# conroi/lcpc

Hardware: AMD Instinct MI355X
Metric: field-elements committed/sec (whole node), Ligero 2^26 coeffs (higher is better)
Workload: dtype u32 limbs (255-bit prime field Ft255, Montgomery form)

## Files before the change

### lcpc_amd/csrc/ntt_l9s.hip

```cpp
#include "kernels.h"
#include "ntt_ln_dev.h"

namespace lcpc {

namespace {

template <bool M2> struct Tw { LN<9> b0, b1; };
template <> struct Tw<false> { LN<9> b0; };
template <bool M2, u32 NV> LCPC_DEV Tw<M2> tw_get(const u32* blk, u32 period, u32 variant, u32 jl) {
  using FT = LnField<FT255>;
  Tw<M2> t;
  if constexpr (M2) {
    t.b0 = pack_get<FT, 2 * NV>(blk, period, variant, jl);
    t.b1 = pack_get<FT, 2 * NV>(blk, period, NV + variant, jl);
  } else {
    t.b0 = pack_get<FT, NV>(blk, period, variant, jl);
  }
  return t;
}
template <bool M2> LCPC_DEV LN<9> tw_mul(const LN<9>& x, const Tw<M2>& w) {
  if constexpr (M2) return ln::mul2<LnField<FT255>>(x, w.b0, w.b1);
  else return ln::mul<LnField<FT255>>(x, w.b0);
}

template <int S, int LTJ, bool FIRST, bool MID, bool NF, bool M2>
__global__ void __launch_bounds__(256, 4) ntt_pass_l9s_kernel(NttPassArgs a, const u32* __restrict__ pack, NttPackInfo pi) {
  using FT = LnField<FT255>;
  constexpr int NL = 8, LT = S + LTJ, LBT = LTJ;
  constexpr bool LAST = !FIRST;
  static_assert(LT == 10, "1024-element tiles: one radix-4 quad (two radix-2 pairs) per thread and round");
  static_assert(FIRST || (LTJ == 0 && S % 2 == 0), "the last pass works on contiguous tiles and ends with the trivial stages k-2, k-1");
  static_assert(NF || !M2, "the two-table multiply serves the pure / coset form only");
  using SH = Shape<S, LBT>;
  using SP = PureShape<S>;
  constexpr int RU = NF ? (FIRST ? SP::RU : -1) : SH::RU;
  constexpr int RC = NF && FIRST ? SP::RC : -1;
  constexpr bool SWZD = NF ? (LAST || SP::RU >= 0) : RU >= 0;
  auto SWZ = [](u32 e) -> u32 {
    if constexpr (NF && LAST) return e ^ (((e >> 4) & 3u) * 5u);
    else if constexpr (NF && FIRST && SWZD && LBT == 2) return e ^ ((((e >> 4) ^ (e >> 6)) & 3u) << 2);
    else if constexpr (SWZD) return e ^ ((e >> 4) & 15u);
    else return e;
  };
  extern __shared__ __attribute__((aligned(16))) u32 lds[];
  constexpr u32 T = 1u << LT;
  u32* nqp = lds + (size_t)T * 9;
  const u32 k = a.log_n;
  const u32 tiles_per_row = 1u << (k - LT);
  u64 row;
  u32 tile;
  if (FIRST && a.tile_group) {
    const u32 lg = a.tile_group;
    const u32 xcd = blockIdx.x & 7u;
    const u64 qq = blockIdx.x >> 3;
    const u32 sub = (u32)qq & ((1u << lg) - 1);
    const u64 q2 = qq >> lg;
    tile = (((u32)(q2 / a.n_rows) * 8u + xcd) << lg) | sub;
    row = q2 % a.n_rows;
  } else if (tiles_per_row >= 8) {
    const u32 xcd = blockIdx.x & 7u;
    const u64 qq = blockIdx.x >> 3;
    tile = (u32)(qq / a.n_rows) * 8u + xcd;
    row = qq % a.n_rows;
  } else {
    row = blockIdx.x / tiles_per_row;
    tile = blockIdx.x % tiles_per_row;
  }
  const u32 tid = threadIdx.x;
  mem_phase(true);
  const u32 lb = FIRST ? k - S : 0u;
  auto gindex = [&](u32 e) -> u32 {
    if constexpr (FIRST) return ((e >> LBT) << lb) | (tile << LTJ) | (e & ((1u << LBT) - 1));
    else return (tile << S) | e;
  };
  const bool canon = a.roots29c != nullptr && ((u32)row & a.canon_row_mask) == 0;
  for (u32 i = tid; i < 64 * 12; i += 256) nqp[i] = 0u - a.qp29[i];
  const u32* src = a.src + row * a.src_stride * NL;
  constexpr bool DIRECT = !(LAST && MID);
  LN<9> xin[4];
  if constexpr (LAST && MID) {
    const uint4* t4 = reinterpret_cast<const uint4*>(a.mid + (row << k) * 9 + (size_t)tile * (9 * T));
    uint4* l4 = reinterpret_cast<uint4*>(lds);
    if constexpr (SWZD) {
#pragma unroll
      for (u32 i = tid; i < 2 * T; i += 256) l4[(i & ~(T - 1)) | SWZ(i & (T - 1))] = t4[i];
#pragma unroll
      for (u32 i = tid; i < T / 4; i += 256) {
        const uint4 v = t4[2 * T + i];
        const u32 b = 8 * T + SWZ(4 * i);
        lds[b] = v.x; lds[b ^ 1u] = v.y; lds[b ^ 2u] = v.z; lds[b ^ 3u] = v.w;
      }
    } else {
#pragma unroll
    for (u32 i = tid; i < 9 * T / 4; i += 256) l4[i] = t4[i];
    }
  } else {
#pragma unroll
  for (u32 it = 0; it < 4; it++) {
    const u32 e = tid + 256u * it;
    const u32 g = gindex(e);
    Fe<NL> v;
    if constexpr (FIRST) {
      v = (g < a.n_valid && row * a.src_stride + g < a.n_src_total) ? fe_load<NL>(src + (size_t)g * NL) : fe_zero<NL>();
      if (a.copy_dst != nullptr && g < a.n_valid) fe_store<NL>(a.copy_dst + (row * a.src_stride + g) * NL, v);
    } else {
      v = fe_load<NL>(src + (size_t)g * NL);
    }
    xin[it] = ln::from_packed<FT>(v);
  }
  __builtin_amdgcn_sched_barrier(0);
  }
  const u32* cls_pack = pack + (size_t)(FIRST != NF ? tile : 0u) * pi.class_words;
  const bool blk0_tile = (FIRST || tile == 0) && a.blk0_gone == 0;
  LN<9> k32;
#pragma unroll
  for (int i = 0; i < 9; i++) k32.v[i] = i == 0 ? 32u : 0u;
  const bool zero_hi = FIRST && a.n_valid <= (1ull << (k - 1));
  if constexpr (!DIRECT) __syncthreads();

  if constexpr (SH::U0 == 1) {
    constexpr u32 half = 1u << (S - 1 + LBT);
    const u32* blk = cls_pack + pi.round_off[0];
#pragma unroll
    for (u32 pp = 0; pp < 2; pp++) {
      const u32 e1 = tid + 256u * pp;
      const Tw<M2> w = NF ? tw_get<M2, 2>(blk, 1u << (S - 1), canon ? 1u : 0u, e1 >> LBT) : tw_get<M2, 2>(blk, SH::period2, canon ? 1u : 0u, e1);
      const LN<9> x = DIRECT ? xin[pp] : planes_get<FT>(lds, T, SWZ(e1));
      if (pp == 0) mem_phase(false);
      const bool cvs = NF && canon && SH::NR4 <= 1;
      if (zero_hi) {
        if constexpr (DIRECT) planes_put<FT>(lds, T, SWZ(e1), cvs ? ln::mul<FT>(x, k32) : x);
        planes_put<FT>(lds, T, SWZ(e1 + half), tw_mul<M2>(x, w));
      } else {
        const LN<9> y = DIRECT ? xin[pp + 2] : planes_get<FT>(lds, T, SWZ(e1 + half));
        LN<9> sum = ln::add(x, y);
        ln::normalize<FT>(sum);
        planes_put<FT>(lds, T, SWZ(e1), cvs ? ln::mul<FT>(sum, k32) : sum);
        planes_put<FT>(lds, T, SWZ(e1 + half), tw_mul<M2>(ln::sub(x, y), w));
      }
    }
    mem_phase(true);
    __syncthreads();
  }

  const u32 q = tid;
  if constexpr (NF && LAST) {
#pragma unroll
    for (int r = 0; r < 5; r++) {
      const int hb = 9 - 2 * r;
      const u32 D = 1u << (hb - 1);
      const u32 m = q >> (hb - 1);
      const u32 e0 = (m << (hb + 1)) | (q & (D - 1));
      const bool from_regs = DIRECT && r == 0;
      LN<9> x0 = from_regs ? xin[0] : planes_get<FT>(lds, T, SWZ(e0));
      const LN<9> x1 = from_regs ? xin[1] : planes_get<FT>(lds, T, SWZ(e0 + D));
      const LN<9> x2 = from_regs ? xin[2] : planes_get<FT>(lds, T, SWZ(e0 + 2 * D)), x3 = from_regs ? xin[3] : planes_get<FT>(lds, T, SWZ(e0 + 3 * D));
      LN<9> p1, p2, p3;
      if (r < 2) {
        const u32 sb = r == 0 ? 0u : (u32)__builtin_amdgcn_readfirstlane(tid >> 6);
        const u32* wu = cls_pack + pi.u_off + ((u32)r * 4 + sb) * (3 * U_SLOT<FT>);
        mem_phase(false);
        if (!from_regs) ln::clamp_apply<FT>(x0, ln::clamp_row<FT>(nqp, ln::clamp_q<FT>(x0.v[8])));
        p2 = ln::mul_u<FT>(x2, wu + U_SLOT<FT>);
        p1 = ln::mul_u<FT>(x1, wu);
        p3 = ln::mul_u<FT>(x3, wu + 2 * U_SLOT<FT>);
      } else {
        const u32* blk = cls_pack + pi.round_off[r];
        const Tw<M2> w1 = tw_get<M2, 3>(blk, coset_sets(r), 0, m), w2 = tw_get<M2, 3>(blk, coset_sets(r), 1, m);
        const Tw<M2> w3 = tw_get<M2, 3>(blk, coset_sets(r), 2, m);
        mem_phase(false);
        ln::clamp_apply<FT>(x0, ln::clamp_row<FT>(nqp, ln::clamp_q<FT>(x0.v[8])));
        p2 = tw_mul<M2>(x2, w2);
        p1 = tw_mul<M2>(x1, w1);
        p3 = tw_mul<M2>(x3, w3);
      }
      const LN<9> s02 = ln::add(x0, p2), d02 = ln::sub(x0, p2), s13 = ln::add(p1, p3);
      LN<9> y0 = ln::add(s02, s13), y1 = ln::sub(s02, s13);
      ln::normalize<FT>(y0);
      const LN<9> t = ln::mul_u<FT>(ln::sub(p1, p3), a.wq_w);
      LN<9> y2 = ln::add(d02, t), y3 = ln::sub(d02, t);
      if (r == 0 || r == 4) { ln::normalize<FT>(y1); ln::normalize<FT>(y2); ln::normalize<FT>(y3); }
      mem_phase(true);
      if (r < 4) {
        planes_put<FT>(lds, T, SWZ(e0), y0);
        planes_put<FT>(lds, T, SWZ(e0 + D), y1);
        planes_put<FT>(lds, T, SWZ(e0 + 2 * D), y2);
        planes_put<FT>(lds, T, SWZ(e0 + 3 * D), y3);
        __syncthreads();
      } else {
        u32* dstq = a.dst + row * a.dst_stride * NL + (size_t)((tile << S) | e0) * NL;
        LN<9> cc[4] = {y0, y1, y2, y3};
#pragma unroll
        for (int c = 0; c < 4; c++) {
          LN<9> x = cc[c];
          ln::clamp_apply<FT>(x, ln::clamp_row<FT>(nqp, ln::clamp_q<FT>(x.v[8])));
          u32 w[8];
          ln::to_packed<FT>(w, x.v);
          Fe<NL> v;
#pragma unroll
          for (int i = 0; i < 8; i++) v.v[i] = w[i];
          if (__any((int)(x.v[8] >= FT::limb(8)))) v = fe_reduce_once<8>(w);
          fe_store<NL>(dstq + (size_t)c * NL, v);
        }
      }
    }
    return;
  }
#pragma unroll
  for (int r = 0; r < SH::NR4; r++) {
    const int u = SH::U0 + 2 * r, hb = S - u - 1;
    const bool last_two = LAST && (r == SH::NR4 - 1);
    const bool triv = NF && FIRST && (r == SH::NR4 - 1);
    const u32 lp = q & ((1u << LBT) - 1), j = q >> LBT;
    const u32 i0 = ((j >> (hb - 1)) << (hb + 1)) | (j & ((1u << (hb - 1)) - 1));
    const u32 e0 = (i0 << LBT) | lp;
    constexpr u32 one = 1u;
    const u32 dq = one << (hb - 1 + LBT);
    const u32 period = NF ? one << (hb - 1) : one << (hb - 1 + LBT);
    const u32 jl = NF ? j & (period - 1) : q & (period - 1);
    const u32* blk = cls_pack + pi.round_off[SH::U0 + r];
    if (triv) {
      const bool fr = DIRECT && SH::U0 == 0 && r == 0;
      const LN<9> x0 = fr ? xin[0] : planes_get<FT>(lds, T, SWZ(e0)), x1 = fr ? xin[1] : planes_get<FT>(lds, T, SWZ(e0 + dq));
      const LN<9> x2 = fr ? xin[2] : planes_get<FT>(lds, T, SWZ(e0 + 2 * dq)), x3 = fr ? xin[3] : planes_get<FT>(lds, T, SWZ(e0 + 3 * dq));
      mem_phase(false);
      const LN<9> b0 = ln::add(x0, x2), b1 = ln::add(x1, x3);
      LN<9> c0 = ln::add(b0, b1), c1 = ln::sub(b0, b1);
      const LN<9> b2 = ln::sub(x0, x2);
      const LN<9> t = ln::mul_u<FT>(ln::sub(x1, x3), a.wq_w);
      LN<9> c2 = ln::add(b2, t), c3 = ln::sub(b2, t);
      ln::normalize<FT>(c1); ln::normalize<FT>(c2); ln::normalize<FT>(c3);
      if (RC < 0 && SH::U0 == 0 && canon) {
        ln::normalize<FT>(c0);
        c0 = ln::mul<FT>(c0, k32); c1 = ln::mul<FT>(c1, k32); c2 = ln::mul<FT>(c2, k32); c3 = ln::mul<FT>(c3, k32);
      } else if (fr) {
        ln::normalize<FT>(c0);
      } else {
        ln::clamp_apply<FT>(c0, ln::clamp_row<FT>(nqp, ln::clamp_q<FT>(c0.v[8])));
      }
      planes_put<FT>(lds, T, SWZ(e0), c0);
      planes_put<FT>(lds, T, SWZ(e0 + dq), c1);
      planes_put<FT>(lds, T, SWZ(e0 + 2 * dq), c2);
      planes_put<FT>(lds, T, SWZ(e0 + 3 * dq), c3);
      mem_phase(true);
      __syncthreads();
      continue;
    }
    if constexpr (RU >= 0) {
      if (r >= RU && !last_two) {
        const u32 wv = __builtin_amdgcn_readfirstlane(tid >> 6);
        const u32 qu = NF ? (((((tid & 63u) >> LBT) << 2) | wv) << LBT) | (tid & ((1u << LBT) - 1)) : ((tid & 63u) << 2) | wv;
        const u32 lpu = qu & ((1u << LBT) - 1), ju = qu >> LBT;
        const u32 iu = ((ju >> (hb - 1)) << (hb + 1)) | (ju & ((1u << (hb - 1)) - 1));
        const u32 eu = (iu << LBT) | lpu;
        const u32* wu = cls_pack + pi.u_off + ((r - RU) * 4 + wv) * (3 * U_SLOT<FT>);
        const LN<9> x0 = planes_get<FT>(lds, T, SWZ(eu)), x1 = planes_get<FT>(lds, T, SWZ(eu + dq));
        const LN<9> x2 = planes_get<FT>(lds, T, SWZ(eu + 2 * dq)), x3 = planes_get<FT>(lds, T, SWZ(eu + 3 * dq));
        mem_phase(false);
        const LN<9> b0 = ln::add(x0, x2), b1 = ln::add(x1, x3);
        LN<9> c0 = ln::add(b0, b1);
        ln::clamp_apply<FT>(c0, ln::clamp_row<FT>(nqp, ln::clamp_q<FT>(c0.v[8])));
        planes_put<FT>(lds, T, SWZ(eu), c0);
        LN<9> d1 = ln::sub(b0, b1);
        ln::normalize<FT>(d1);
        planes_put<FT>(lds, T, SWZ(eu + dq), ln::mul_u<FT>(d1, wu + 2 * U_SLOT<FT>));
        const LN<9> b2 = ln::mul_u<FT>(ln::sub(x0, x2), wu);
        const LN<9> b3 = ln::mul_u<FT>(ln::sub(x1, x3), wu + U_SLOT<FT>);
        LN<9> c2 = ln::add(b2, b3);
        if constexpr (NF) ln::clamp_apply<FT>(c2, ln::clamp_row<FT>(nqp, ln::clamp_q<FT>(c2.v[8])));
        else ln::normalize<FT>(c2);
        planes_put<FT>(lds, T, SWZ(eu + 2 * dq), c2);
        planes_put<FT>(lds, T, SWZ(eu + 3 * dq), ln::mul_u<FT>(ln::sub(b2, b3), wu + 2 * U_SLOT<FT>));
        mem_phase(true);
        __syncthreads();
        continue;
      }
    }
    if (u == 0 && zero_hi) {
      const u32 vb = canon ? 3u : 0u;
      const Tw<M2> w0 = tw_get<M2, 6>(blk, period, vb + 0, jl), w3 = tw_get<M2, 6>(blk, period, vb + 1, jl), w2 = tw_get<M2, 6>(blk, period, vb + 2, jl);
      mem_phase(false);
      const bool cv0 = NF && canon && r == RC;
      if (a.n_valid <= (1ull << (k - 2))) {
        const LN<9> x0 = DIRECT ? xin[0] : planes_get<FT>(lds, T, SWZ(e0));
        if constexpr (DIRECT) planes_put<FT>(lds, T, SWZ(e0), cv0 ? ln::mul<FT>(x0, k32) : x0);
        planes_put<FT>(lds, T, SWZ(e0 + dq), tw_mul<M2>(x0, w2));
        planes_put<FT>(lds, T, SWZ(e0 + 2 * dq), tw_mul<M2>(x0, w0));
        planes_put<FT>(lds, T, SWZ(e0 + 3 * dq), tw_mul<M2>(x0, w3));
      } else {
        const LN<9> x0 = DIRECT ? xin[0] : planes_get<FT>(lds, T, SWZ(e0)), x1 = DIRECT ? xin[1] : planes_get<FT>(lds, T, SWZ(e0 + dq));
        LN<9> c0 = ln::add(x0, x1);
        ln::normalize<FT>(c0);
        planes_put<FT>(lds, T, SWZ(e0), cv0 ? ln::mul<FT>(c0, k32) : c0);
        planes_put<FT>(lds, T, SWZ(e0 + dq), tw_mul<M2>(ln::sub(x0, x1), w2));
        const LN<9> t = ln::mul_u<FT>(x1, a.wq_w);
        planes_put<FT>(lds, T, SWZ(e0 + 2 * dq), tw_mul<M2>(ln::add(x0, t), w0));
        planes_put<FT>(lds, T, SWZ(e0 + 3 * dq), tw_mul<M2>(ln::sub(x0, t), w3));
      }
      mem_phase(true);
      __syncthreads();
      continue;
    }
    const bool from_regs = DIRECT && SH::U0 == 0 && r == 0;
    const LN<9> x0 = from_regs ? xin[0] : planes_get<FT>(lds, T, SWZ(e0)), x1 = from_regs ? xin[1] : planes_get<FT>(lds, T, SWZ(e0 + dq));
    const LN<9> x2 = from_regs ? xin[2] : planes_get<FT>(lds, T, SWZ(e0 + 2 * dq)), x3 = from_regs ? xin[3] : planes_get<FT>(lds, T, SWZ(e0 + 3 * dq));
    mem_phase(false);
    const LN<9> b0 = ln::add(x0, x2), b1 = ln::add(x1, x3);
    LN<9> c0 = ln::add(b0, b1);
    if (last_two) {
      ln::normalize<FT>(c0);
      LN<9> c1 = ln::sub(b0, b1);
      const LN<9> b2 = ln::sub(x0, x2);
      const LN<9> b3 = ln::mul_u<FT>(ln::sub(x1, x3), a.wq_w);
      LN<9> c2 = ln::add(b2, b3);
      LN<9> c3 = ln::sub(b2, b3);
      ln::normalize<FT>(c1); ln::normalize<FT>(c2); ln::normalize<FT>(c3);
      mem_phase(true);
      u32* dstq = a.dst + row * a.dst_stride * NL + (size_t)((tile << S) | e0) * NL;
      LN<9> cc[4] = {c0, c1, c2, c3};
#pragma unroll
      for (int c = 0; c < 4; c++) {
        LN<9> x = cc[c];
        ln::clamp_apply<FT>(x, ln::clamp_row<FT>(nqp, ln::clamp_q<FT>(x.v[8])));
        u32 w[8];
        ln::to_packed<FT>(w, x.v);
        Fe<NL> v;
#pragma unroll
        for (int i = 0; i < 8; i++) v.v[i] = w[i];
        if (__any((int)(x.v[8] >= FT::limb(8)))) v = fe_reduce_once<8>(w);
        fe_store<NL>(dstq + (size_t)c * NL, v);
      }
      return;
    } else {
      if (from_regs) ln::normalize<FT>(c0);
      else ln::clamp_apply<FT>(c0, ln::clamp_row<FT>(nqp, ln::clamp_q<FT>(c0.v[8])));
      planes_put<FT>(lds, T, SWZ(e0), c0);
      const bool blk0c = NF ? canon && q < dq : canon && blk0_tile && q < period && (RU < 0 || r < RU);
      if constexpr (NF ? RC >= 0 : RU >= 1) {
        if (r == (NF ? RC : RU - 1) && blk0c) {
          planes_put<FT>(lds, T, SWZ(e0), ln::mul<FT>(c0, k32));
        }
      }
      const u32 vb = blk0c ? 3u : 0u;
      if constexpr (M2) {
        const Tw<M2> w2 = tw_get<M2, 6>(blk, period, vb + 2, jl), w0 = tw_get<M2, 6>(blk, period, vb + 0, jl);
        const LN<9> d1 = ln::sub(b0, b1);
        const LN<9> d13 = ln::sub(x1, x3), e2 = ln::sub(x0, x2);
        planes_put<FT>(lds, T, SWZ(e0 + dq), tw_mul<M2>(d1, w2));
        __builtin_amdgcn_sched_barrier(0);
        const Tw<M2> w3 = tw_get<M2, 6>(blk, period, vb + 1, jl);
        const LN<9> t = ln::mul_u<FT>(d13, a.wq_w);
        planes_put<FT>(lds, T, SWZ(e0 + 2 * dq), tw_mul<M2>(ln::add(e2, t), w0));
        planes_put<FT>(lds, T, SWZ(e0 + 3 * dq), tw_mul<M2>(ln::sub(e2, t), w3));
      } else {
      const Tw<M2> w0 = tw_get<M2, 6>(blk, period, vb + 0, jl), w3 = tw_get<M2, 6>(blk, period, vb + 1, jl);
      const Tw<M2> w2 = tw_get<M2, 6>(blk, period, vb + 2, jl);
      const LN<9> d1 = ln::sub(b0, b1);
      planes_put<FT>(lds, T, SWZ(e0 + dq), tw_mul<M2>(d1, w2));
      const LN<9> t = ln::mul_u<FT>(ln::sub(x1, x3), a.wq_w);
      const LN<9> e2 = ln::sub(x0, x2);
      planes_put<FT>(lds, T, SWZ(e0 + 2 * dq), tw_mul<M2>(ln::add(e2, t), w0));
      planes_put<FT>(lds, T, SWZ(e0 + 3 * dq), tw_mul<M2>(ln::sub(e2, t), w3));
      }
    }
    mem_phase(true);
    __syncthreads();
  }

  if constexpr (FIRST && MID) {
    u32* mrow = a.mid + (row << k) * 9;
#pragma unroll
    for (u32 e = tid; e < T; e += 256) {
      const u32 e2 = (tile << LTJ) | (e & ((1u << LBT) - 1));
      u32* t = mrow + (size_t)(e >> LBT) * (9 * T);
      const LN<9> x = planes_get<FT>(lds, T, SWZ(e));
      *reinterpret_cast<uint4*>(t + (size_t)e2 * 4) = make_uint4(x.v[0], x.v[1], x.v[2], x.v[3]);
      *reinterpret_cast<uint4*>(t + (size_t)(T + e2) * 4) = make_uint4(x.v[4], x.v[5], x.v[6], x.v[7]);
      t[(size_t)8 * T + e2] = x.v[8];
    }
    return;
  }
  if constexpr (FIRST) {
  u32* dst = a.dst + row * a.dst_stride * NL;
#pragma unroll
  for (u32 e = tid; e < T; e += 256) {
    const u32 g = gindex(e);
    LN<9> x = planes_get<FT>(lds, T, SWZ(e));
    ln::clamp_apply<FT>(x, ln::clamp_row<FT>(nqp, ln::clamp_q<FT>(x.v[8])));
    u32 w[8];
    ln::to_packed<FT>(w, x.v);
    Fe<NL> v;
#pragma unroll
    for (int i = 0; i < 8; i++) v.v[i] = w[i];
    fe_store<NL>(dst + (size_t)g * NL, v);
  }
  }
}

template <int S, int LTJ, bool FIRST, bool MID, bool NF, bool M2>
hipError_t launch_tm(const NttPassArgs& a, const u32* pack, const NttPackInfo& pi, hipStream_t st) {
  constexpr int LT = S + LTJ;
  const u64 tiles = ((u64)1 << (a.log_n - LT)) * a.n_rows;
  const size_t lds_bytes = (((size_t)1 << LT) * 9 + 64 * LnField<FT255>::STRIDE) * 4;
  hipError_t e = hipFuncSetAttribute(reinterpret_cast<const void*>(&ntt_pass_l9s_kernel<S, LTJ, FIRST, MID, NF, M2>),
                                     hipFuncAttributeMaxDynamicSharedMemorySize, (int)lds_bytes);
  if (e != hipSuccess) return e;
  hipLaunchKernelGGL((ntt_pass_l9s_kernel<S, LTJ, FIRST, MID, NF, M2>), dim3((unsigned)tiles), dim3(256), lds_bytes, st, a, pack, pi);
  return hipGetLastError();
}
template <int S, int LTJ, bool FIRST>
hipError_t launch_t(const NttPassArgs& a, const u32* pack, const NttPackInfo& pi, hipStream_t st) {
  if (pi.mul2) {
    if constexpr (ntt_l9s_mul2_supported(S, FIRST)) { if (a.form) return a.mid ? launch_tm<S, LTJ, FIRST, true, true, true>(a, pack, pi, st) : launch_tm<S, LTJ, FIRST, false, true, true>(a, pack, pi, st); }
    return hipErrorInvalidValue;
  }
  if (a.form) return a.mid ? launch_tm<S, LTJ, FIRST, true, true, false>(a, pack, pi, st) : launch_tm<S, LTJ, FIRST, false, true, false>(a, pack, pi, st);
  return a.mid ? launch_tm<S, LTJ, FIRST, true, false, false>(a, pack, pi, st) : launch_tm<S, LTJ, FIRST, false, false, false>(a, pack, pi, st);
}

}

bool ntt_l9s3_supported(uint32_t log_n) { return log_n >= 21 && log_n <= 26; }

bool ntt_l9s_supported(uint32_t log_n, uint32_t n_passes, int log_tile) { return n_passes == 2 && log_tile == 10 && log_n >= 11 && log_n <= 20; }

#define L9S_FIRST_CASES(X) X(1) X(2) X(3) X(4) X(5) X(6) X(7) X(8) X(9) X(10)

hipError_t launch_ntt_pass_l9s(const NttPassArgs& a, bool first, const uint32_t* pack, const NttPackInfo& pi, hipStream_t st) {
  if (!first) {
    if (a.s != 10 || a.log_tj != 0 || a.t0 + a.s != a.log_n) return hipErrorInvalidValue;
    if (a.mont_prefix) return hipErrorInvalidValue;
    return launch_t<10, 0, false>(a, pack, pi, st);
  }
  if (a.t0 != 0 || a.s + a.log_tj != 10 || (a.s + 10 != a.log_n && a.s + 20 != a.log_n)) return hipErrorInvalidValue;
  if (a.form && a.s + 10 != a.log_n) return hipErrorInvalidValue;
  if (a.tile_group && ((1u << (a.log_n - 10)) >> a.tile_group) < 8) return hipErrorInvalidValue;
  switch (a.s) {
#define X(SV) case SV: return launch_t<SV, 10 - SV, true>(a, pack, pi, st);
    L9S_FIRST_CASES(X)
#undef X
  }
  return hipErrorInvalidValue;
}

}
```

### lcpc_amd/csrc/ntt_ln_dev.h

```cpp
#pragma once
#include "field_ln.h"

namespace lcpc {

template <int S, int LBT> struct Shape {
  static constexpr int U0 = S & 1;
  static constexpr int NR4 = S / 2;
  static constexpr u32 period2 = 1u << (S - 1 + LBT);
  static constexpr u32 period4(int r) { return 1u << (S - U0 - 2 * r - 2 + LBT); }
  static constexpr int RU = NR4 >= 4 ? 3 : -1;
  static constexpr int NRU = RU < 0 ? 0 : NR4 - RU;
};
template <int S> struct PureShape {
  static constexpr int U0 = S & 1;
  static constexpr int NR4 = S / 2;
  static constexpr u32 sets(int r) { return 1u << (S - U0 - 2 * r - 2); }
  static constexpr int RU = NR4 >= 3 ? NR4 - 2 : -1;
  static constexpr int RC = NR4 >= 3 ? NR4 - 3 : (NR4 == 2 ? 0 : -1);
};
constexpr u32 coset_sets(int r) { return 1u << (2 * r); }

template <class FT> constexpr u32 U_SLOT = (FT::N * FT::N + 31) & ~31u;
template <class FT> constexpr u32 U_ALIGN = FT::N == 9 ? 4u : 16u;

template <class FT, class C = u32> LCPC_DEV LN<FT::N> planes_get(const u32* base, C cnt, u32 e) {
  constexpr int N = FT::N;
  LN<N> r;
  if constexpr (N == 3) {
    const uint2 a = *reinterpret_cast<const uint2*>(base + (size_t)e * 2);
    r.v[0] = a.x; r.v[1] = a.y; r.v[2] = base[(size_t)cnt * 2 + e];
  } else {
    const uint4 a = *reinterpret_cast<const uint4*>(base + (size_t)e * 4);
    r.v[0] = a.x; r.v[1] = a.y; r.v[2] = a.z; r.v[3] = a.w;
    if constexpr (N == 5) {
      r.v[4] = base[(size_t)cnt * 4 + e];
    } else if constexpr (N == 7) {
      const uint2 b = *reinterpret_cast<const uint2*>(base + (size_t)cnt * 4 + (size_t)e * 2);
      r.v[4] = b.x; r.v[5] = b.y; r.v[6] = base[(size_t)cnt * 6 + e];
    } else {
      const uint4 b = *reinterpret_cast<const uint4*>(base + ((size_t)cnt + e) * 4);
      r.v[4] = b.x; r.v[5] = b.y; r.v[6] = b.z; r.v[7] = b.w; r.v[8] = base[(size_t)cnt * 8 + e];
    }
  }
  return r;
}
template <class FT, class C = u32> LCPC_DEV void planes_put(u32* base, C cnt, u32 e, const LN<FT::N>& x) {
  constexpr int N = FT::N;
  if constexpr (N == 3) {
    *reinterpret_cast<uint2*>(base + (size_t)e * 2) = make_uint2(x.v[0], x.v[1]);
    base[(size_t)cnt * 2 + e] = x.v[2];
  } else {
    *reinterpret_cast<uint4*>(base + (size_t)e * 4) = make_uint4(x.v[0], x.v[1], x.v[2], x.v[3]);
    if constexpr (N == 5) {
      base[(size_t)cnt * 4 + e] = x.v[4];
    } else if constexpr (N == 7) {
      *reinterpret_cast<uint2*>(base + (size_t)cnt * 4 + (size_t)e * 2) = make_uint2(x.v[4], x.v[5]);
      base[(size_t)cnt * 6 + e] = x.v[6];
    } else {
      *reinterpret_cast<uint4*>(base + ((size_t)cnt + e) * 4) = make_uint4(x.v[4], x.v[5], x.v[6], x.v[7]);
      base[(size_t)cnt * 8 + e] = x.v[8];
    }
  }
}

template <class FT> LCPC_DEV LN<FT::N> tab_entry(const u32* tab, u32 idx) {
  if constexpr (FT::STRIDE == 12) {
    return ln::load_limbs<FT::N>(tab + (size_t)idx * 12);
  } else {
    LN<FT::N> t;
#pragma unroll
    for (int k = 0; k < FT::N; k++) t.v[k] = tab[(size_t)idx * FT::STRIDE + k];
    return t;
  }
}

template <class FT, u32 NV> LCPC_DEV LN<FT::N> pack_get(const u32* blk, u32 period, u32 variant, u32 jl) {
  if constexpr (FT::N == 9) {
    const char* base = reinterpret_cast<const char*>(blk);
    const uint4 a = *reinterpret_cast<const uint4*>(base + (((variant * 2 + 0) * period + jl) << 4));
    const uint4 b = *reinterpret_cast<const uint4*>(base + (((variant * 2 + 1) * period + jl) << 4));
    const u32 c = *reinterpret_cast<const u32*>(base + ((NV * 2 * period * 4 + variant * period + jl) << 2));
    LN<9> t;
    t.v[0] = a.x; t.v[1] = a.y; t.v[2] = a.z; t.v[3] = a.w; t.v[4] = b.x; t.v[5] = b.y; t.v[6] = b.z; t.v[7] = b.w; t.v[8] = c;
    return t;
  } else {
    return planes_get<FT>(blk, NV * period, variant * period + jl);
  }
}
template <class FT, u32 NV> LCPC_DEV void pack_put(u32* blk, u32 period, u32 variant, u32 jl, const LN<FT::N>& x) {
  if constexpr (FT::N == 9) {
    *reinterpret_cast<uint4*>(blk + ((size_t)(variant * 2 + 0) * period + jl) * 4) = make_uint4(x.v[0], x.v[1], x.v[2], x.v[3]);
    *reinterpret_cast<uint4*>(blk + ((size_t)(variant * 2 + 1) * period + jl) * 4) = make_uint4(x.v[4], x.v[5], x.v[6], x.v[7]);
    blk[(size_t)NV * 2 * period * 4 + (size_t)variant * period + jl] = x.v[8];
  } else {
    planes_put<FT>(blk, NV * period, variant * period + jl, x);
  }
}

}
```

Measured before the change: 7.540 billion.

## Drop redundant normalizes before clamp-store and fuse trivial final round with global store

Removes normalize calls on outputs that are immediately clamped and stored, relying on clamp_store to bring values into range. Adds a path where the trivial (twiddle-free) last radix-4 round in non-MID configurations writes directly to global memory via gindex instead of going through LDS and another pass. Factors the clamp/pack/reduce/store sequence into a shared clamp_store helper. This saves ALU work and an LDS round trip, but correctness depends on clamp bounds tolerating unnormalized inputs, and the extra path without reduction must still yield canonical values.

```diff
diff --git a/lcpc_amd/csrc/ntt_l9s.hip b/lcpc_amd/csrc/ntt_l9s.hip
--- a/lcpc_amd/csrc/ntt_l9s.hip
+++ b/lcpc_amd/csrc/ntt_l9s.hip
@@ -176,10 +176,10 @@
       }
       const LN<9> s02 = ln::add(x0, p2), d02 = ln::sub(x0, p2), s13 = ln::add(p1, p3);
       LN<9> y0 = ln::add(s02, s13), y1 = ln::sub(s02, s13);
-      ln::normalize<FT>(y0);
+      if (r < 4) ln::normalize<FT>(y0);
       const LN<9> t = ln::mul_u<FT>(ln::sub(p1, p3), a.wq_w);
       LN<9> y2 = ln::add(d02, t), y3 = ln::sub(d02, t);
-      if (r == 0 || r == 4) { ln::normalize<FT>(y1); ln::normalize<FT>(y2); ln::normalize<FT>(y3); }
+      if (r == 0) { ln::normalize<FT>(y1); ln::normalize<FT>(y2); ln::normalize<FT>(y3); }
       mem_phase(true);
       if (r < 4) {
         planes_put<FT>(lds, T, SWZ(e0), y0);
@@ -189,19 +189,10 @@
         __syncthreads();
       } else {
         u32* dstq = a.dst + row * a.dst_stride * NL + (size_t)((tile << S) | e0) * NL;
-        LN<9> cc[4] = {y0, y1, y2, y3};
-#pragma unroll
-        for (int c = 0; c < 4; c++) {
-          LN<9> x = cc[c];
-          ln::clamp_apply<FT>(x, ln::clamp_row<FT>(nqp, ln::clamp_q<FT>(x.v[8])));
-          u32 w[8];
-          ln::to_packed<FT>(w, x.v);
-          Fe<NL> v;
-#pragma unroll
-          for (int i = 0; i < 8; i++) v.v[i] = w[i];
-          if (__any((int)(x.v[8] >= FT::limb(8)))) v = fe_reduce_once<8>(w);
-          fe_store<NL>(dstq + (size_t)c * NL, v);
-        }
+        clamp_store<FT, true>(dstq, y0, nqp);
+        clamp_store<FT, true>(dstq + (size_t)1 * NL, y1, nqp);
+        clamp_store<FT, true>(dstq + (size_t)2 * NL, y2, nqp);
+        clamp_store<FT, true>(dstq + (size_t)3 * NL, y3, nqp);
       }
     }
     return;
@@ -229,6 +220,20 @@
       const LN<9> b2 = ln::sub(x0, x2);
       const LN<9> t = ln::mul_u<FT>(ln::sub(x1, x3), a.wq_w);
       LN<9> c2 = ln::add(b2, t), c3 = ln::sub(b2, t);
+      if constexpr (!MID && SH::NR4 >= 1) {
+        if (RC < 0 && SH::U0 == 0 && canon) {
+          ln::normalize<FT>(c0); ln::normalize<FT>(c1); ln::normalize<FT>(c2); ln::normalize<FT>(c3);
+          c0 = ln::mul<FT>(c0, k32); c1 = ln::mul<FT>(c1, k32); c2 = ln::mul<FT>(c2, k32); c3 = ln::mul<FT>(c3, k32);
+        }
+        if constexpr (SH::U0 == 0 && SH::NR4 == 1) __syncthreads();
+        mem_phase(true);
+        u32* dstq = a.dst + row * a.dst_stride * NL;
+        clamp_store<FT, false>(dstq + (size_t)gindex(e0) * NL, c0, nqp);
+        clamp_store<FT, false>(dstq + (size_t)gindex(e0 + dq) * NL, c1, nqp);
+        clamp_store<FT, false>(dstq + (size_t)gindex(e0 + 2 * dq) * NL, c2, nqp);
+        clamp_store<FT, false>(dstq + (size_t)gindex(e0 + 3 * dq) * NL, c3, nqp);
+        return;
+      }
       ln::normalize<FT>(c1); ln::normalize<FT>(c2); ln::normalize<FT>(c3);
       if (RC < 0 && SH::U0 == 0 && canon) {
         ln::normalize<FT>(c0);
@@ -308,28 +313,17 @@
     const LN<9> b0 = ln::add(x0, x2), b1 = ln::add(x1, x3);
     LN<9> c0 = ln::add(b0, b1);
     if (last_two) {
-      ln::normalize<FT>(c0);
       LN<9> c1 = ln::sub(b0, b1);
       const LN<9> b2 = ln::sub(x0, x2);
       const LN<9> b3 = ln::mul_u<FT>(ln::sub(x1, x3), a.wq_w);
       LN<9> c2 = ln::add(b2, b3);
       LN<9> c3 = ln::sub(b2, b3);
-      ln::normalize<FT>(c1); ln::normalize<FT>(c2); ln::normalize<FT>(c3);
       mem_phase(true);
       u32* dstq = a.dst + row * a.dst_stride * NL + (size_t)((tile << S) | e0) * NL;
-      LN<9> cc[4] = {c0, c1, c2, c3};
-#pragma unroll
-      for (int c = 0; c < 4; c++) {
-        LN<9> x = cc[c];
-        ln::clamp_apply<FT>(x, ln::clamp_row<FT>(nqp, ln::clamp_q<FT>(x.v[8])));
-        u32 w[8];
-        ln::to_packed<FT>(w, x.v);
-        Fe<NL> v;
-#pragma unroll
-        for (int i = 0; i < 8; i++) v.v[i] = w[i];
-        if (__any((int)(x.v[8] >= FT::limb(8)))) v = fe_reduce_once<8>(w);
-        fe_store<NL>(dstq + (size_t)c * NL, v);
-      }
+      clamp_store<FT, true>(dstq, c0, nqp);
+      clamp_store<FT, true>(dstq + (size_t)1 * NL, c1, nqp);
+      clamp_store<FT, true>(dstq + (size_t)2 * NL, c2, nqp);
+      clamp_store<FT, true>(dstq + (size_t)3 * NL, c3, nqp);
       return;
     } else {
       if (from_regs) ln::normalize<FT>(c0);
diff --git a/lcpc_amd/csrc/ntt_ln_dev.h b/lcpc_amd/csrc/ntt_ln_dev.h
--- a/lcpc_amd/csrc/ntt_ln_dev.h
+++ b/lcpc_amd/csrc/ntt_ln_dev.h
@@ -63,6 +63,20 @@
   }
 }
 
+template <class FT, bool REDUCE> LCPC_DEV void clamp_store(u32* dst, LN<FT::N> x, const u32* nqp) {
+  constexpr int N = FT::N, NL = FT::NL;
+  ln::clamp_apply<FT>(x, ln::clamp_row<FT>(nqp, ln::clamp_q<FT>(x.v[N - 1])));
+  u32 w[NL];
+  ln::to_packed<FT>(w, x.v);
+  Fe<NL> v;
+#pragma unroll
+  for (int i = 0; i < NL; i++) v.v[i] = w[i];
+  if constexpr (REDUCE) {
+    if (__any((int)(x.v[N - 1] >= FT::limb(N - 1)))) v = fe_reduce_once<NL>(w);
+  }
+  fe_store<NL>(dst, v);
+}
+
 template <class FT> LCPC_DEV LN<FT::N> tab_entry(const u32* tab, u32 idx) {
   if constexpr (FT::STRIDE == 12) {
     return ln::load_limbs<FT::N>(tab + (size_t)idx * 12);
```

Measured after the change: 7.651 billion (median of 6 runs). 1.5% higher.
